# taha-kms/CLASSMATE-RAG

Measured on AMD Instinct MI355X. Metric: hybrid queries/sec + recall@10 vs reference, 10M×768 chunks, 1/2/4/8 GPU, higher is better.
Workload: dtype fp32-accurate E5 (K10 f16x3 MFMA) + int8/f16/f64 dense + f64 BM25

## Files before the change

classmate-rag_amd/classmate_hip/_lib.py:

```python
from __future__ import annotations

import ctypes as C
import os
from pathlib import Path

try:
    import torch
except Exception:
    torch = None

LIB_NAME = "libclassmate_hip.so"
LIB_PATH = Path(os.environ.get("CLASSMATE_HIP_LIB", Path(__file__).with_name(LIB_NAME)))

CM_OK, CM_EINVAL, CM_ENOMEM, CM_EDEVICE, CM_EZERODIV, CM_EUNSUPPORTED = 0, -1, -2, -3, -4, -5
CM_FOP_EQ, CM_FOP_NE, CM_FOP_BITS, CM_FOP_TRUE, CM_FOP_FALSE, CM_FOP_AND, CM_FOP_OR, CM_FOP_NOT = range(1, 9)
CM_FILTER_MAX_OPS, CM_FILTER_MAX_SOURCES = 64, 16
CM_DTYPE_F32, CM_DTYPE_BF16, CM_DTYPE_F16, CM_DTYPE_I32, CM_DTYPE_I64 = 0, 1, 2, 3, 4

if not LIB_PATH.exists():
    raise ImportError(
        f"{LIB_PATH} not found: build the HIP extension first "
        f"(python -c 'import __graft_entry__ as g; g.build()' or make -C classmate-rag_amd)")

lib = C.CDLL(str(LIB_PATH), mode=C.RTLD_GLOBAL)
# ... 66 lines not shown
    "cm_bm25_append": (c_int, c_vp, c_vp, c_vp, c_i64, c_i32),
    "cm_bm25_append_dev": (c_int, c_vp, c_vp, c_vp, c_i64, c_i64, c_i32, c_vp),
    "cm_bm25_remove": (c_int, c_vp, c_vp, c_i64),
    "cm_bm25_remove_dev": (c_int, c_vp, c_vp, c_vp),
    "cm_bm25_replace": (c_int, c_vp, c_vp, c_i64, c_vp, c_vp, c_i32),
    "cm_bm25_replace_dev": (c_int, c_vp, c_vp, c_i64, c_vp, c_vp, c_i64, c_i32, c_vp),
    "cm_bm25_num_docs": (c_i64, c_vp),
    "cm_bm25_num_postings": (c_i64, c_vp),
    "cm_bm25_stats": (c_int, c_vp, P(c_i64), P(c_i64), P(c_f64), P(c_f64)),
    "cm_bm25_export": (c_int, c_vp, c_vp, c_vp, c_vp, c_vp, c_vp),
    "cm_bm25_set_head_policy": (c_int, c_vp, c_f64, c_i64),
    "cm_bm25_num_head_terms": (c_i32, c_vp),
    "cm_bm25_set_path": (c_int, c_vp, c_i32),
    "cm_bm25_workspace_rescored": (c_i32, c_vp, c_i32, c_i32, c_i32, c_vp),
    "cm_bm25_last_rescored": (c_i32, c_vp),
    "cm_bm25_term_stats": (c_int, c_vp, c_vp, c_vp),
    "cm_bm25_set_stats": (c_int, c_vp, c_vp, c_i32, c_i64, c_i64, c_f64),
    "cm_bm25_search": (c_int, c_vp, c_vp, c_vp, c_i32, c_i32, c_vp, c_vp, c_vp, c_vp),
    "cm_bm25_search_lists": (c_int, c_vp, c_vp, c_vp, c_i32, c_i32, c_vp, c_i32, c_vp, c_vp, c_vp, c_vp),
    "cm_bm25_search_lists_dev": (c_int, c_vp, c_vp, c_vp, c_i32, c_i32, c_vp, c_i32, c_vp, c_vp, c_vp, c_vp, c_vp,
                                 c_vp),
    "cm_bm25_last_eps_filters": (c_i32, c_vp),
    "cm_bm25_workspace_items": (c_i64, c_vp, c_i32, c_i32, c_i32, c_vp, c_vp, c_i64),
    "cm_bm25_workspace_subblocks": (c_i64, c_vp, c_i32, c_i32, c_i32, c_vp, c_vp, c_i64),
    "cm_bm25_timing_drain_block": (c_i32, c_vp, c_vp, c_i32),
    "cm_bm25_search_idf": (c_int, c_vp, c_vp, c_vp, c_i32, c_i32, c_vp, c_vp, c_f64, c_i64, c_vp, c_vp, c_vp),
    "cm_bm25_search_workspace": (c_i64, c_vp, c_i32, c_i32, c_i32),
    "cm_bm25_search_dev": (c_int, c_vp, c_vp, c_vp, c_i32, c_i32, c_i32, c_vp, c_vp, c_vp, c_i64, c_vp),
    "cm_bm25_search_dev_gated": (c_int, c_vp, c_vp, c_vp, c_i32, c_i32, c_i32, c_vp, c_vp, c_vp, c_i64, c_vp, c_vp),
    "cm_bm25_prepare_filtered": (c_int, c_vp, c_i64),
    "cm_bm25_filter_stats_dev": (c_int, c_vp, c_vp, c_vp, c_i32, c_vp, c_vp, c_vp),
    "cm_bm25_filter_term_stats_dev": (c_int, c_vp, c_vp, c_vp, c_vp, c_vp),
    "cm_bm25_filter_eps": (c_int, c_vp, c_vp, P(c_f64)),
    "cm_bm25_filter_eps_multi": (c_int, c_vp, c_vp, c_i32, c_vp),
    "cm_bm25_last_eps_passes": (c_i32, c_vp),
    "cm_bm25_search_stats_dev": (c_int, c_vp, c_vp, c_vp, c_i32, c_i32, c_i32, c_vp, c_vp, c_vp, c_vp, c_vp, c_vp,
                                 c_vp, c_vp, c_i64, c_vp),
    "cm_bm25_search_filtered_dev": (c_int, c_vp, c_vp, c_vp, c_i32, c_i32, c_i32, c_vp, c_vp, c_vp, c_vp, c_vp,
                                    c_vp, c_i64, c_vp),
    "cm_mmr": (c_int, c_vp, c_vp, c_vp, c_i32, c_i32, c_i32, c_i32, c_f64, c_vp),
    "cm_mmr_dev": (c_int, c_vp, c_vp, c_vp, c_i32, c_i32, c_i32, c_i32, c_f64, c_vp, c_vp),
    "cm_rrf_fuse": (c_int, c_vp, c_vp, c_i32, c_vp, c_i32, c_vp, c_vp, P(c_i32)),
    "cm_rrf_merge": (c_int, c_vp, c_vp, c_vp, c_i32, c_vp, c_vp, c_vp, c_i32, c_i32, c_f64, c_f64, c_i32, c_i32,
                     c_vp, c_vp, c_vp, c_vp, c_vp, c_vp),
    "cm_rrf_pool_prep_dev": (c_int, c_vp, c_vp, c_i32, c_vp, c_i32, c_vp, c_i32, c_i32, c_vp, c_vp, c_vp, c_vp,
                             c_vp),
# ... 58 lines not shown
```

classmate-rag_amd/classmate_hip/engine.py:

```python
from __future__ import annotations

import ctypes as C
import os
from typing import Optional, Sequence

import numpy as np

from . import _lib as L

try:
    import torch
except Exception:
    torch = None


def default_device() -> int:
    env = os.environ.get("CM_DEVICE")
    if env:
        return int(env)
    if torch is not None and torch.cuda.is_available():
        return torch.cuda.current_device()
    return 0


# ... 459 lines not shown
        L.check(L.fn["cm_bm25_timing"](self._h, int(bool(enable))), "cm_bm25_timing")

    def timing_drain(self, cap: int = 4096) -> list:
        buf = np.zeros(cap, np.float32)
        n = int(L.fn["cm_bm25_timing_drain"](self._h, L.ptr(buf), int(cap)))
        if n < 0:
            raise RuntimeError(L.last_error())
        return buf[:min(n, cap)].tolist()

    def timing_drain_block(self, cap: int = 4096) -> list:
        buf = np.zeros(cap, np.float32)
        n = int(L.fn["cm_bm25_timing_drain_block"](self._h, L.ptr(buf), int(cap)))
        if n < 0:
            raise RuntimeError(L.last_error())
        return buf[:min(n, cap)].tolist()

    def workspace_items(self, nq: int, total_terms: int, k: int, workspace, cap: int = 1 << 22) -> np.ndarray:
        buf = np.zeros(cap, np.uint64)
        n = int(L.fn["cm_bm25_workspace_items"](self._h, int(nq), int(total_terms), int(k), L.ptr(workspace),
                                                 L.ptr(buf), int(cap)))
        if n < 0:
            raise RuntimeError(L.last_error() or "no planned items (full path?)")
        return buf[:min(n, cap)]

    def workspace_subblocks(self, nq: int, total_terms: int, k: int, workspace, cap: int = 1 << 22) -> np.ndarray:
        buf = np.zeros(cap, np.uint64)
        n = int(L.fn["cm_bm25_workspace_subblocks"](self._h, int(nq), int(total_terms), int(k), L.ptr(workspace),
                                                     L.ptr(buf), int(cap)))
        if n < 0:
            raise RuntimeError(L.last_error() or "no planned items (full path?)")
        return buf[:min(n, cap)]

    @property
    def num_head_terms(self) -> int:
        return int(L.fn["cm_bm25_num_head_terms"](self._h))

    def term_stats(self):
        df = np.zeros(max(self.vocab, 1), np.int32)
        fk = np.zeros(max(self.vocab, 1), np.uint64)
        L.check(L.fn["cm_bm25_term_stats"](self._h, L.ptr(df), L.ptr(fk)), "cm_bm25_term_stats")
        return df[: self.vocab], fk[: self.vocab]

    def set_stats(self, idf: np.ndarray, n_live: int, sum_len: int, eps: float):
        v = _c(idf, np.float64)
        L.check(L.fn["cm_bm25_set_stats"](self._h, L.ptr(v), int(v.shape[0]), int(n_live), int(sum_len), float(eps)),
                "cm_bm25_set_stats")
# ... 526 lines not shown
```

classmate-rag_amd/csrc/cm_bm25.hip:

```cpp
#include "cm_common.h"
#include "cm_row_lists.h"

#include <hipcub/hipcub.hpp>

#include <algorithm>
#include <cmath>
#include <cstdlib>
#include <numeric>
#include <vector>

namespace cm {

constexpr int kRange = 1024;
constexpr int kBmThreads = 256;
constexpr int kBoundsGroup = 8;
constexpr int kMergeThreads = 1024;
constexpr int kMergePer = 16;
constexpr int kTermLanesQd = 16;

__device__ inline int64_t lhead(int q, int64_t r, int64_t nr) { return (int64_t)q * nr + r; }
__host__ __device__ inline int64_t lheads_total(int nq, int64_t nr) { return (int64_t)nq * nr; }
__device__ inline int64_t lslot(int q, int64_t r, int64_t nr, int64_t nl, int k, int j) {
  return j == 0 ? lhead(q, r, nr) : nl + ((int64_t)q * nr + r) * (k - 1) + (j - 1);
}
// ... 201 lines not shown
  return __longlong_as_double(((uint64_t)hi << 32) | lo);
}
__device__ inline uint64_t readlane_u64(uint64_t v, int j) {
  const uint32_t lo = __builtin_amdgcn_readlane((uint32_t)v, j);
  const uint32_t hi = __builtin_amdgcn_readlane((uint32_t)(v >> 32), j);
  return ((uint64_t)hi << 32) | lo;
}
__device__ inline void wave_lds_sync() {
  __builtin_amdgcn_fence(__ATOMIC_RELEASE, "wavefront");
  __builtin_amdgcn_wave_barrier();
  __builtin_amdgcn_fence(__ATOMIC_ACQUIRE, "wavefront");
}
template <typename P>
__device__ inline int first_ge(const P *__restrict__ a, int lo, int hi, int32_t target) {
  while (lo < hi) {
    const int mid = (lo + hi) >> 1;
    if (a[mid] < target) lo = mid + 1;
    else hi = mid;
  }
  return lo;
}

template <typename TF>
__global__ void __launch_bounds__(kBmThreads) __attribute__((amdgpu_waves_per_eu(K2_WAVES_PER_EU)))
    bm25_range_kernel(const int32_t *__restrict__ q_terms, const int32_t *__restrict__ q_off, int nq,
                      const double *__restrict__ q_idf, const int64_t *__restrict__ bounds, int nr, int rpw,
                      const int32_t *__restrict__ post_doc, const TF *__restrict__ post_tf,
                      const int32_t *__restrict__ head_id, const uint8_t *__restrict__ headtf, int64_t npad,
                      const int32_t *__restrict__ dl, const uint32_t *__restrict__ live,
                      const uint32_t *__restrict__ allow, int64_t ndocs, const double *__restrict__ avgdl_p,
                      const double *__restrict__ lut, int lut_dmin, int k,
                      uint64_t *__restrict__ cand_key, uint32_t *__restrict__ cand_row,
                      unsigned long long *__restrict__ thr_key, const uint8_t *__restrict__ need, int32_t vocab,
                      int dbg) {
  __shared__ double s_lut[kLutW * kLutTF];
#ifndef CM_ABLATION
  dbg = 0;
#endif
  __shared__ int32_t s_pdoc[kBmThreads / 64][kTailCapW];
  __shared__ uint16_t s_ptf[kBmThreads / 64][kTailCapW];
  __shared__ uint64_t s_keys[kBmThreads / 64][16 * 64];
  const double avgdl = *avgdl_p;
  for (int i = threadIdx.x; i < kLutW * kLutTF; i += kBmThreads) s_lut[i] = lut[i];
  __syncthreads();
  const int lane = threadIdx.x & 63;
  const int wave = threadIdx.x >> 6;
  const int nb = gridDim.x;
  const int b = blockIdx.x;
  const int per = nb >> 3, rem = nb & 7, x = b & 7, y = b >> 3;
  const int lb = (x < rem ? x * (per + 1) : rem * (per + 1) + (x - rem) * per) + y;
  const int nqg = (nq + kQPerWave - 1) / kQPerWave;
  const int wid = lb * (kBmThreads / 64) + wave;
  const int qg = wid % nqg;
  const int q0 = qg * kQPerWave;
  const int rg = wid / nqg;
  const int r0 = rg * rpw, r1 = min(r0 + rpw, nr);
  if (r0 >= r1) return;
  const int nqw = min(kQPerWave, nq - q0);
  auto need_at = [&](int r) -> uint32_t {
    return need ? (uint32_t)__builtin_amdgcn_readfirstlane((int)need[(int64_t)qg * nr + r]) : 0xfu;
  };
  if (need) {
    uint32_t any = 0;
    for (int r = r0; r < r1; ++r) any |= need_at(r);
    if (!any) return;
  }
  int32_t *pdoc = s_pdoc[wave];
  uint16_t *ptf = s_ptf[wave];
  uint64_t *keys = s_keys[wave];
  const int64_t bstride = nr + 1;
  const int my_q = lane / kTermLanes, my_j = lane % kTermLanes;
  int my_tb = 0, my_L = 0;
  if (my_q < nqw) {
    my_tb = q_off[q0 + my_q];
    my_L = q_off[q0 + my_q + 1] - my_tb;
  }
  const bool has_term = my_q < nqw && my_j < my_L;
  const int my_i = my_tb + my_j;
  int32_t my_t = -1, my_h = -1;
  double my_idf = 0.0;
  int64_t my_lo = 0, my_hi = 0;
  if (has_term) {
    my_t = q_terms[my_i];
    if (my_t >= vocab) my_t = -1;
    my_idf = q_idf[my_i];
    my_h = (my_t >= 0 && head_id) ? head_id[my_t] : -1;
    if (my_h < 0) {
      my_lo = bounds[(int64_t)my_i * bstride + r0];
      my_hi = bounds[(int64_t)my_i * bstride + r0 + 1];
    }
  }
  const bool walk = has_term && my_h < 0;
// ... 238 lines not shown
          for (int u = 0; u < 16; ++u) {
            const uint64_t key = keys[u * 64 + lane];
            if (key < bk) {
              bk = key;
              bu = u;
            }
          }
          br = bk == kEmptyKey ? 0xffffffffu : (uint32_t)db + (uint32_t)bu;
        }
      }
      if (lane == 0 && i < k) {
        const int64_t o = lslot(qi, r, nr, lheads_total(nq, nr), k, i);
        cand_key[o] = kEmptyKey;
        cand_row[o] = 0xffffffffu;
      }
      if (i == k && lane == 0 && last < T) atomicMin(thr_key + qi, (unsigned long long)last);
    }
    my_lo = nx_lo;
    my_hi = nx_hi;
    wave_lds_sync();
  }
}

#include "cm_bm25_prune.inc"

__global__ void bm25_head_fill_kernel(const int32_t *__restrict__ head_terms, int nhead,
                                      const int64_t *__restrict__ term_off, const int32_t *__restrict__ post_doc,
                                      const uint16_t *__restrict__ post_tf, uint8_t *__restrict__ headtf,
                                      int64_t npad) {
  const int h = blockIdx.y;
  if (h >= nhead) return;
  const int32_t t = head_terms[h];
  const int64_t lo = term_off[t], hi = term_off[t + 1];
  uint8_t *row = headtf + (int64_t)h * npad;
  for (int64_t p = lo + (int64_t)blockIdx.x * blockDim.x + threadIdx.x; p < hi; p += (int64_t)gridDim.x * blockDim.x)
    row[post_doc[p]] = (uint8_t)post_tf[p];
}

__global__ void bm25_dl_hist_kernel(const int32_t *__restrict__ dl, int64_t ndocs, uint32_t *__restrict__ hist) {
  for (int64_t i = (int64_t)blockIdx.x * blockDim.x + threadIdx.x; i < ndocs; i += (int64_t)gridDim.x * blockDim.x) {
    const int32_t d = dl[i];
    if (d >= 0 && d < 65536) atomicAdd(hist + d, 1u);
  }
}

__global__ void bm25_head_sat_kernel(const int32_t *__restrict__ cand, int ncand, const int64_t *__restrict__ term_off,
// ... 564 lines not shown
  return e ? atoi(e) : 0;
}
#else
int bm25_debug_flags() { return 0; }
#endif

struct BmWs {
  unsigned long long *thr;
  double *lut;
  double *q_idf;
  int64_t *bounds;
  uint64_t *cand_key;
  uint32_t *cand_row;
  uint8_t *need;
  uint64_t *items;
  uint64_t *items_sm;
  uint8_t *qcand;
  int32_t *qd_code;
  double *qd_idf;
  int32_t *qd_tb;
  int32_t *qd_len;
  int32_t *qd_term;
  uint32_t *item_count;
  double *avgdl;
  int64_t *stats;
  int64_t *df;
  size_t total;
};

BmWs bm_ws_layout(const cm_bm25 *h, int nq, int total_terms, int k, void *base) {
  BmWs w{};
  char *p = reinterpret_cast<char *>(base);
  const int64_t nr = std::max<int64_t>(1, ceil_div(h->ndocs, kRange));
  size_t off = 0;
  w.thr = reinterpret_cast<unsigned long long *>(p + off);
  off += round_up((int64_t)std::max(nq, 1) * 8, 256);
  w.lut = reinterpret_cast<double *>(p + off);
  off += round_up((int64_t)kLutW * kLutTF * 8, 256);
  w.q_idf = reinterpret_cast<double *>(p + off);
  off += round_up((int64_t)std::max(total_terms, 1) * 8, 256);
  w.bounds = reinterpret_cast<int64_t *>(p + off);
  off += round_up((int64_t)std::max(total_terms, 1) * (nr + 1) * 8, 256);
  const int64_t n_slots = lheads_total(nq, nr) + (int64_t)nq * nr * (k - 1);
  w.cand_key = reinterpret_cast<uint64_t *>(p + off);
  off += round_up(n_slots * 8, 256);
  w.cand_row = reinterpret_cast<uint32_t *>(p + off);
  off += round_up(n_slots * 4, 256);
  w.need = reinterpret_cast<uint8_t *>(p + off);
  off += round_up(ceil_div(std::max(nq, 1), kQPerWave) * nr, 256);
  w.items = reinterpret_cast<uint64_t *>(p + off);
  off += round_up((int64_t)std::max(nq, 1) * nr * 8, 256);
  w.items_sm = reinterpret_cast<uint64_t *>(p + off);
  off += round_up((int64_t)std::max(nq, 1) * nr * 8, 256);
  w.item_count = reinterpret_cast<uint32_t *>(p + off);
  off += 256;
  w.qcand = reinterpret_cast<uint8_t *>(p + off);
  off += round_up(std::max(total_terms, 1), 256);
  w.avgdl = reinterpret_cast<double *>(p + off);
  off += 256;
  w.stats = reinterpret_cast<int64_t *>(p + off);
  off += 256;
  w.df = reinterpret_cast<int64_t *>(p + off);
  off += round_up((int64_t)std::max(total_terms, 1) * 8, 256);
  w.qd_code = reinterpret_cast<int32_t *>(p + off);
  off += round_up((int64_t)std::max(nq, 1) * kTermLanes * 4, 256);
  w.qd_idf = reinterpret_cast<double *>(p + off);
  off += round_up((int64_t)std::max(nq, 1) * kTermLanes * 8, 256);
  w.qd_tb = reinterpret_cast<int32_t *>(p + off);
  off += round_up((int64_t)std::max(nq, 1) * 4, 256);
  w.qd_len = reinterpret_cast<int32_t *>(p + off);
  off += round_up((int64_t)std::max(nq, 1) * 4, 256);
  w.qd_term = reinterpret_cast<int32_t *>(p + off);
  off += round_up((int64_t)std::max(nq, 1) * kTermLanes * 4, 256);
  w.total = off;
  return w;
}

#ifndef K2A_RPW
// ... 10 lines not shown
                     const uint32_t *allow_dev, const BmWs &w, double *score_dev, int64_t *row_dev, hipStream_t st,
                     hipEvent_t gate = nullptr) {
  int rc;
  const double *avgdl = w.avgdl;
  const int nr = (int)std::max<int64_t>(1, ceil_div(h->ndocs, kRange));
  if (nr > kMergePer * kMergeThreads) CM_FAIL(CM_EUNSUPPORTED, "BM25 shard too large (> 16.7M docs)");
  const int ngroups = (nr + 1 + kBoundsGroup - 1) / kBoundsGroup;
  const int64_t nb = (int64_t)total_terms * ngroups;
  const bool prune = h->path != 1 && !(bm25_debug_flags() & 4);
  if (nq > 0) {
    hipLaunchKernelGGL(bm25_qcand_kernel, dim3((unsigned)ceil_div(nq, 256)), dim3(256), 0, st, q_terms_dev, q_off_dev,
                       nq, h->vocab, h->nhead ? h->head_id.as<int32_t>() : (const int32_t *)nullptr,
                       h->term_off.as<int64_t>(), (int)prune, w.qcand, w.q_idf, prune ? w.qd_code : nullptr,
                       w.qd_idf, w.qd_tb, w.qd_len, w.qd_term);
    CM_HIP(hipGetLastError());
  }
  if (nb > 0) {
    hipLaunchKernelGGL(bm25_bounds_kernel, dim3((unsigned)ceil_div(nb, 256)), dim3(256), 0, st, q_terms_dev,
                       total_terms, h->vocab, nr, h->term_off.as<int64_t>(), h->post_doc.as<int32_t>(), w.qcand,
                       w.bounds);
    CM_HIP(hipGetLastError());
  }
  CM_HIP(hipMemsetAsync(w.thr, 0xff, (size_t)nq * 8, st));
  if (prune && nq > 0 && env_knob("CM_BM25_TSEED", true)) {
    hipLaunchKernelGGL(bm25_tseed_kernel, dim3((unsigned)nq), dim3(kSeedThreads), 0, st, nq, k, w.qd_code,
                       w.qd_idf, w.qd_len, w.qd_term, h->term_off.as<int64_t>(), h->post_doc.as<int32_t>(),
                       h->post_tf.as<uint16_t>(), h->headtf.as<uint8_t>(), h->npad, h->dl.as<int32_t>(),
                       h->live.as<uint32_t>(), allow_dev, avgdl, w.thr);
    CM_HIP(hipGetLastError());
  }
  hipLaunchKernelGGL(bm25_lut_kernel, dim3(kLutW * kLutTF / 256), dim3(256), 0, st, (const double *)avgdl, h->lut_dmin,
                     w.lut);
  CM_HIP(hipGetLastError());
  const int64_t nqg = ceil_div(nq, kQPerWave);
  const int rpw = (int)std::min<int64_t>(kMaxRangesPerWave, std::max<int64_t>(1, nqg * nr / (256 * 4 * 24)));
  const int64_t nwaves = nqg * ceil_div(nr, rpw);
  const int64_t nblk = ceil_div(nwaves, kBmThreads / 64);
  const int rpw_a = std::max(1, std::min(rpw, (int)K2A_RPW));
  const int64_t nblk_a = ceil_div(nqg * ceil_div(nr, rpw_a), K2A_W);
  if (nblk > INT32_MAX || nblk_a > INT32_MAX) CM_FAIL(CM_EUNSUPPORTED, "BM25 batch too large");
  const int32_t *head_id = h->nhead ? h->head_id.as<int32_t>() : (const int32_t *)nullptr;
  if (gate) CM_HIP(hipStreamWaitEvent(st, gate, 0));
#if K2A_TRACE
  if (prune) {
    if ((rc = g_k2a_trace_buf.ensure((size_t)nblk_a * K2A_W * 32))) return rc;
    g_k2a_trace_units = nblk_a * K2A_W;
    uint64_t *tp = g_k2a_trace_buf.as<uint64_t>();
    CM_HIP(hipMemsetAsync(tp, 0, (size_t)g_k2a_trace_units * 32, st));
    CM_HIP(hipMemcpyToSymbolAsync(HIP_SYMBOL(g_k2a_trace), &tp, sizeof(tp), 0, hipMemcpyHostToDevice, st));
  }
#endif
  h->timer.begin(st);
  if (prune) {
    hipLaunchKernelGGL(bm25_tail_kernel<uint16_t>, dim3((unsigned)nblk_a), dim3(64 * K2A_W), 0, st, nq, w.bounds, nr,
                       rpw_a, h->post_doc.as<int32_t>(), h->post_tf.as<uint16_t>(), h->headtf.as<uint8_t>(), h->npad,
                       h->dl.as<int32_t>(), h->live.as<uint32_t>(), allow_dev, avgdl, k, w.cand_key, w.cand_row, w.thr,
                       w.need, w.qd_code, w.qd_term, w.qd_idf, w.qd_tb, w.qd_len, bm25_debug_flags());
    h->timer.end(st);
    CM_HIP(hipGetLastError());
    if ((rc = launch_bm25_merge(w.cand_key, w.cand_row, nq, nr, k, score_dev, row_dev, st))) return rc;
    CM_HIP(hipMemsetAsync(w.item_count, 0, 4, st));
    hipLaunchKernelGGL(bm25_plan_kernel, dim3((unsigned)ceil_div(nqg * nr, 256)), dim3(256), 0, st, w.qd_code,
                       w.qd_idf, w.qd_len, nq, (int)(head_id != nullptr), h->head_maxtf.as<uint8_t>(),
                       h->range_mindl.as<int32_t>(), h->blk_maxtf.as<uint8_t>(), h->blk_mindl.as<int32_t>(),
                       (h->nhead && h->maxr_avgdl > 0.0) ? h->blk_maxr.as<uint8_t>() : (const uint8_t *)nullptr,
                       h->maxr_avgdl, nr, (int64_t)nr * (kRange / 64), avgdl, k, score_dev, row_dev, w.need, w.items,
                       w.item_count,
                       (h->nhead && h->maxr_avgdl > 0.0 && !env_knob("CM_BM25_SUB16_OFF", false))
                           ? h->blk16_maxr.as<uint8_t>() : (const uint8_t *)nullptr,
                       w.items_sm);
    CM_HIP(hipGetLastError());
    h->timer_b.begin(st);
    hipLaunchKernelGGL(bm25_block_kernel, dim3(K2B_GRID), dim3(256), 0, st, w.items, w.item_count, w.qd_code,
                       w.qd_idf, w.qd_tb, w.bounds, nr, h->post_doc.as<int32_t>(), h->headtf.as<uint8_t>(), h->npad,
                       h->dl.as<int32_t>(), h->live.as<uint32_t>(), allow_dev, h->ndocs, avgdl, k, score_dev, nq,
                       w.cand_key, w.cand_row, w.items_sm);
    h->timer_b.end(st);
    CM_HIP(hipGetLastError());
  }
  hipLaunchKernelGGL(bm25_range_kernel<uint16_t>, dim3((unsigned)nblk), dim3(kBmThreads), 0, st, q_terms_dev,
                     q_off_dev, nq, w.q_idf, w.bounds, nr, rpw, h->post_doc.as<int32_t>(),
                     h->post_tf.as<uint16_t>(), head_id, h->headtf.as<uint8_t>(), h->npad, h->dl.as<int32_t>(),
                     h->live.as<uint32_t>(), allow_dev, h->ndocs, avgdl, w.lut, h->lut_dmin, k, w.cand_key,
                     w.cand_row, w.thr, prune ? (const uint8_t *)w.need : (const uint8_t *)nullptr, h->vocab,
                     bm25_debug_flags());
  if (!prune) h->timer.end(st);
  CM_HIP(hipGetLastError());
  return launch_bm25_merge(w.cand_key, w.cand_row, nq, nr, k, score_dev, row_dev, st);
}

int32_t count_rescored(cm_bm25 *h, int nq, const BmWs &w, hipStream_t st) {
  const int64_t nr = std::max<int64_t>(1, ceil_div(h->ndocs, kRange));
  const int64_t n = ceil_div(std::max(nq, 1), kQPerWave) * nr;
  std::vector<uint8_t> v((size_t)n);
  uint32_t items = 0;
  if (hipMemcpyAsync(v.data(), w.need, (size_t)n, hipMemcpyDeviceToHost, st) != hipSuccess ||
      hipMemcpyAsync(&items, w.item_count, 4, hipMemcpyDeviceToHost, st) != hipSuccess ||
      hipStreamSynchronize(st) != hipSuccess)
    return -1;
  int64_t c = items;
  for (uint8_t b : v) c += __builtin_popcount(b);
  return (int32_t)std::min<int64_t>(c, INT32_MAX);
}

void bm25_free(cm_bm25 *h) {
  for (DevBuf *b : {&h->term_off, &h->post_doc, &h->post_tf, &h->post_pos, &h->dl, &h->live, &h->idf, &h->ws,
                    &h->qbuf, &h->obuf, &h->allow_buf, &h->tmp, &h->eps_ws, &h->headtf, &h->head_id, &h->head_maxtf,
                    &h->range_mindl, &h->blk_maxtf, &h->blk_mindl, &h->blk_maxr, &h->blk16_maxr})
// ... 440 lines not shown
  return count_rescored(h, nq, w, h->stream);
}

int32_t cm_bm25_last_rescored(cm_bm25 *h) { return h ? h->last_rescored : -1; }

int64_t cm_bm25_workspace_items(cm_bm25 *h, int32_t nq, int32_t total_terms, int32_t k, const void *workspace_dev,
                                uint64_t *items_out, int64_t cap) {
  if (!h || !workspace_dev || nq <= 0 || k <= 0 || cap < 0) return -1;
  if (h->path == 1) return -1;
  DeviceGuard dg(h->dev);
  const BmWs w = bm_ws_layout(h, nq, total_terms, k, const_cast<void *>(workspace_dev));
  uint32_t n = 0;
  if (hipMemcpyAsync(&n, w.item_count, 4, hipMemcpyDeviceToHost, h->stream) != hipSuccess ||
      hipStreamSynchronize(h->stream) != hipSuccess)
    return -1;
  const int64_t m = std::min<int64_t>(n, cap);
  if (m > 0 && items_out &&
      (hipMemcpyAsync(items_out, w.items, (size_t)m * 8, hipMemcpyDeviceToHost, h->stream) != hipSuccess ||
       hipStreamSynchronize(h->stream) != hipSuccess))
    return -1;
  return n;
}

int64_t cm_bm25_workspace_subblocks(cm_bm25 *h, int32_t nq, int32_t total_terms, int32_t k, const void *workspace_dev,
                                    uint64_t *masks_out, int64_t cap) {
  if (!h || !workspace_dev || nq <= 0 || k <= 0 || cap < 0) return -1;
  if (h->path == 1) return -1;
  DeviceGuard dg(h->dev);
  const BmWs w = bm_ws_layout(h, nq, total_terms, k, const_cast<void *>(workspace_dev));
  uint32_t n = 0;
  if (hipMemcpyAsync(&n, w.item_count, 4, hipMemcpyDeviceToHost, h->stream) != hipSuccess ||
      hipStreamSynchronize(h->stream) != hipSuccess)
    return -1;
  const int64_t m = std::min<int64_t>(n, cap);
  if (m > 0 && masks_out &&
      (hipMemcpyAsync(masks_out, w.items_sm, (size_t)m * 8, hipMemcpyDeviceToHost, h->stream) != hipSuccess ||
       hipStreamSynchronize(h->stream) != hipSuccess))
    return -1;
  return n;
}

#if K2A_TRACE
int64_t cm_bm25_k2a_trace(cm_bm25 *h, uint64_t *out, int64_t cap_units) {
  if (!h || !out) return -1;
  DeviceGuard dg(h->dev);
  if (hipDeviceSynchronize() != hipSuccess) return -1;
// ... 357 lines not shown
```

classmate-rag_amd/csrc/cm_bm25_prune.inc:

```

#ifndef K2A_CAP
#define K2A_CAP 320
#endif
#ifndef K2A_SUB
#define K2A_SUB 4
#endif
#ifndef K2B_U
#define K2B_U 2
#endif
#ifndef K2A_WPE
#define K2A_WPE 5
#endif
#ifndef K2A_W
#define K2A_W 1
#endif

#ifndef K2A_TRACE
#define K2A_TRACE 0
#endif
#if K2A_TRACE
__device__ uint64_t *g_k2a_trace;
#endif
typedef uint16_t u16x2_t __attribute__((ext_vector_type(2)));
constexpr int kCandCap = K2A_CAP;
// ... 336 lines not shown
    r += nsub;
  }
#if K2A_TRACE
  if (lane == 0) {
    uint64_t *tr = g_k2a_trace + 4 * (int64_t)wid;
    const uint64_t xcc = __builtin_amdgcn_s_getreg((3 << 11) | 20) & 15u;
    tr[0] = (xcc << 32) | (uint64_t)(wid + 1);
    tr[1] = tr_t0;
    tr[2] = __builtin_amdgcn_s_memrealtime();
    tr[3] = tr_post;
  }
#endif
}

__global__ void __launch_bounds__(256)
    bm25_plan_kernel(const int32_t *__restrict__ qd_code, const double *__restrict__ qd_idf,
                     const int32_t *__restrict__ qd_len, int nq, int has_heads,
                     const uint8_t *__restrict__ head_maxtf, const int32_t *__restrict__ range_mindl,
                     const uint8_t *__restrict__ blk_maxtf, const int32_t *__restrict__ blk_mindl,
                     const uint8_t *__restrict__ blk_maxr, double maxr_avgdl, int nr,
                     int64_t nblk, const double *__restrict__ avgdl_p, int k, const double *__restrict__ top_score,
                     const int64_t *__restrict__ top_row, uint8_t *__restrict__ need, uint64_t *__restrict__ items,
                     uint32_t *__restrict__ item_count, const uint8_t *__restrict__ blk16_maxr,
                     uint64_t *__restrict__ items_sm) {
  const double avgdl = *avgdl_p;
  const bool use_r = blk_maxr != nullptr && avgdl <= maxr_avgdl;
  const float inv_avg = inv_avg_lo(avgdl);
  auto kd_lo = [&](int32_t dlen) __attribute__((always_inline)) { return kd_lo32(dlen, inv_avg); };
  const int nqg = (nq + kQPerWave - 1) / kQPerWave;
  const int64_t gid = (int64_t)blockIdx.x * blockDim.x + threadIdx.x;
  const bool act = gid < (int64_t)nqg * nr;
  const int lane = threadIdx.x & 63;
  uint64_t it[kQPerWave], its[kQPerWave];
  int nit = 0;
  if (act) {
    const int qg = (int)(gid / nr), r = (int)(gid - (int64_t)qg * nr);
    uint32_t m = need[gid];
    const float kd = kd_lo(range_mindl[r]);
    for (int qq = 0; qq < kQPerWave; ++qq) {
      const int q = qg * kQPerWave + qq;
      if (q >= nq) break;
      const uint32_t bit = 1u << qq;
      if (m & bit) continue;
      const double T = top_score[(int64_t)q * k + k - 1];
      if (qd_len[q] > kTermLanes || top_row[(int64_t)q * k + k - 1] < 0 || !(T > 0.0)) {
        m |= bit;
        continue;
      }
      if (!has_heads) continue;
      int32_t hs[kTermLanes];
      float fi[kTermLanes];
      uint32_t mt[kTermLanes];
      {
        const int4 *cp = reinterpret_cast<const int4 *>(qd_code + (int64_t)q * kTermLanes);
        const double2 *ip = reinterpret_cast<const double2 *>(qd_idf + (int64_t)q * kTermLanes);
#pragma unroll
        for (int v = 0; v < kTermLanes / 4; ++v) {
// ... 89 lines not shown
        if ((double)(ubb[b] * kPlanSlack) >= T) bm |= 1u << b;
      uint64_t sm = 0;
#pragma unroll
      for (int b = 0; b < 16; ++b) {
        if (!((bm >> b) & 1u)) continue;
        if (!use_s) {
          sm |= 0xfull << (4 * b);
          continue;
        }
#pragma unroll
        for (int x = 0; x < 4; ++x)
          if ((double)(ubs[4 * b + x] * kPlanSlack) >= T) sm |= 1ull << (4 * b + x);
      }
      uint32_t bms = 0;
#pragma unroll
      for (int b = 0; b < 16; ++b)
        if ((sm >> (4 * b)) & 0xfull) bms |= 1u << b;
      if (bms) {
        its[nit] = sm;
        it[nit++] = ((uint64_t)q << 40) | ((uint64_t)r << 16) | bms;
      }
    }
    need[gid] = (uint8_t)m;
  }
  int incl = nit;
#pragma unroll
  for (int o = 1; o < 64; o <<= 1) {
    const int v = __shfl_up(incl, o);
    if (lane >= o) incl += v;
  }
  const int total = __shfl(incl, 63);
  if (total == 0) return;
  uint32_t base = 0;
  if (lane == 63) base = atomicAdd(item_count, (uint32_t)total);
  base = (uint32_t)__shfl((int)base, 63);
  for (int i = 0; i < nit; ++i) {
    items[base + (uint32_t)(incl - nit + i)] = it[i];
    items_sm[base + (uint32_t)(incl - nit + i)] = its[i];
  }
}

__device__ inline bool k2b_below(const uint32_t (&tfv)[kTermLanes], float fi, float kd, double T, uint64_t headm) {
  float ub = 0.0f;
#pragma unroll
  for (int j = 0; j < kTermLanes; ++j)
    if ((headm >> j) & 1u) ub += __int_as_float(__builtin_amdgcn_readlane(__float_as_int(fi), j)) * ratio_up32(tfv[j], kd);
// ... 456 lines not shown
```

include/classmate_hip.h:

```cpp
#ifndef CLASSMATE_HIP_H
#define CLASSMATE_HIP_H

#include <stddef.h>
#include <stdint.h>

#ifdef __cplusplus
extern "C" {
#endif

#define CM_OK 0
#define CM_EINVAL (-1)
#define CM_ENOMEM (-2)
#define CM_EDEVICE (-3)
#define CM_EZERODIV (-4)
#define CM_EUNSUPPORTED (-5)

#define CM_DTYPE_F32 0
#define CM_DTYPE_BF16 1
#define CM_DTYPE_F16 2
#define CM_DTYPE_I32 3
#define CM_DTYPE_I64 4

const char *cm_last_error(void);
int cm_version(void);
// ... 72 lines not shown
int cm_bm25_append(cm_bm25 *h, const int32_t *term_ids, const int64_t *doc_off, int64_t n_new, int32_t vocab);
int cm_bm25_append_dev(cm_bm25 *h, const int32_t *term_ids_dev, const int64_t *doc_off_dev, int64_t n_new,
                       int64_t ntokens, int32_t vocab, void *stream);
int cm_bm25_remove(cm_bm25 *h, const int64_t *rows, int64_t n_rows);
int cm_bm25_remove_dev(cm_bm25 *h, const uint32_t *remove_bits_dev, void *stream);
int cm_bm25_replace(cm_bm25 *h, const int64_t *rows, int64_t n_rows, const int32_t *term_ids, const int64_t *doc_off,
                    int32_t vocab);
int cm_bm25_replace_dev(cm_bm25 *h, const int64_t *rows_dev, int64_t n_rows, const int32_t *term_ids_dev,
                        const int64_t *doc_off_dev, int64_t ntokens, int32_t vocab, void *stream);
int64_t cm_bm25_num_docs(cm_bm25 *h);
int64_t cm_bm25_num_postings(cm_bm25 *h);
int cm_bm25_stats(cm_bm25 *h, int64_t *n_live, int64_t *sum_len, double *avgdl, double *eps);
int cm_bm25_set_head_policy(cm_bm25 *h, double min_df_frac, int64_t max_bytes);
int32_t cm_bm25_num_head_terms(cm_bm25 *h);
#define CM_BM25_FULL 1
#define CM_BM25_PRUNED 2
int cm_bm25_set_path(cm_bm25 *h, int32_t kind);
int32_t cm_bm25_workspace_rescored(cm_bm25 *h, int32_t nq, int32_t total_terms, int32_t k, const void *workspace_dev);
int32_t cm_bm25_last_rescored(cm_bm25 *h);
int64_t cm_bm25_workspace_items(cm_bm25 *h, int32_t nq, int32_t total_terms, int32_t k, const void *workspace_dev,
                                uint64_t *items_out, int64_t cap);
int64_t cm_bm25_workspace_subblocks(cm_bm25 *h, int32_t nq, int32_t total_terms, int32_t k, const void *workspace_dev,
                                    uint64_t *masks_out, int64_t cap);
int cm_bm25_timing(cm_bm25 *h, int32_t enable);
int32_t cm_bm25_timing_drain(cm_bm25 *h, float *ms_out, int32_t cap);
int32_t cm_bm25_timing_drain_block(cm_bm25 *h, float *ms_out, int32_t cap);
int cm_bm25_export(cm_bm25 *h, int64_t *term_off, int32_t *post_doc, uint16_t *post_tf, uint32_t *post_pos,
                   int32_t *dl);
int cm_bm25_term_stats(cm_bm25 *h, int32_t *df_out, uint64_t *first_out);
int cm_bm25_set_stats(cm_bm25 *h, const double *idf, int32_t vocab, int64_t n_live, int64_t sum_len, double eps);
int cm_bm25_search(cm_bm25 *h, const int32_t *q_terms, const int32_t *q_off, int32_t nq, int32_t k,
                   const uint32_t *allow_bits, double *out_score, int64_t *out_row, int32_t *out_n);
int cm_bm25_search_lists(cm_bm25 *h, const int32_t *q_terms, const int32_t *q_off, int32_t nq, int32_t k,
                         const uint32_t *allow_bits, int32_t n_filters, const int32_t *filter_of,
                         double *out_score, int64_t *out_row, int32_t *out_n);
int cm_bm25_search_lists_dev(cm_bm25 *h, const int32_t *q_terms, const int32_t *q_off, int32_t nq, int32_t k,
                             const uint32_t *allow_bits, int32_t n_filters, const int32_t *filter_of, double *eps_io,
                             double *score_dev, int64_t *row_dev, int32_t *out_n, void *stream);
int32_t cm_bm25_last_eps_filters(cm_bm25 *h);
int cm_bm25_search_idf(cm_bm25 *h, const int32_t *q_terms, const int32_t *q_off, int32_t nq, int32_t k,
                       const uint32_t *allow_bits, const double *q_idf, double avgdl, int64_t n_cand,
                       double *out_score, int64_t *out_row, int32_t *out_n);
int64_t cm_bm25_search_workspace(cm_bm25 *h, int32_t nq, int32_t total_terms, int32_t k);
int cm_bm25_search_dev(cm_bm25 *h, const int32_t *q_terms_dev, const int32_t *q_off_dev, int32_t nq,
                       int32_t total_terms, int32_t k, double *score_dev, int64_t *row_dev,
                       void *workspace_dev, int64_t workspace_bytes, void *stream);
// ... 95 lines not shown
```

Before: 35220.

## Compact needed BM25 ranges into a work list for the range kernel

The plan kernel now appends every (query-group, range) pair whose need mask is nonzero to a compact device list via wave-ballot atomics. The range kernel gains a LIST variant that launches a fixed grid and has waves grid-stride over only the listed pairs, instead of launching one wave per pair and early-exiting on empty ones. This is meant to remove launch and scheduling cost for the many pruned-away ranges and to balance work better. In exchange it adds an atomic counter, extra workspace, and one range per list entry, which loses the multi-range-per-wave batching.

After: 35390 (median of 6 runs). About the same (+0.5%).

```diff
diff --git a/classmate-rag_amd/classmate_hip/_lib.py b/classmate-rag_amd/classmate_hip/_lib.py
--- a/classmate-rag_amd/classmate_hip/_lib.py
+++ b/classmate-rag_amd/classmate_hip/_lib.py
@@ -112,6 +112,7 @@
                                  c_vp),
     "cm_bm25_last_eps_filters": (c_i32, c_vp),
     "cm_bm25_workspace_items": (c_i64, c_vp, c_i32, c_i32, c_i32, c_vp, c_vp, c_i64),
+    "cm_bm25_workspace_need_ranges": (c_i64, c_vp, c_i32, c_i32, c_i32, c_vp, c_vp, c_vp, c_i64),
     "cm_bm25_workspace_subblocks": (c_i64, c_vp, c_i32, c_i32, c_i32, c_vp, c_vp, c_i64),
     "cm_bm25_timing_drain_block": (c_i32, c_vp, c_vp, c_i32),
     "cm_bm25_search_idf": (c_int, c_vp, c_vp, c_vp, c_i32, c_i32, c_vp, c_vp, c_f64, c_i64, c_vp, c_vp, c_vp),
diff --git a/classmate-rag_amd/classmate_hip/engine.py b/classmate-rag_amd/classmate_hip/engine.py
--- a/classmate-rag_amd/classmate_hip/engine.py
+++ b/classmate-rag_amd/classmate_hip/engine.py
@@ -505,6 +505,17 @@
         if n < 0:
             raise RuntimeError(L.last_error() or "no planned items (full path?)")
         return buf[:min(n, cap)]
+
+    def workspace_need_ranges(self, nq: int, total_terms: int, k: int, workspace, detail: bool = False):
+        nqg, nr = (int(nq) + 3) // 4, max(1, (self.num_docs + 1023) // 1024)
+        lst = np.zeros(nqg * nr, np.uint32)
+        need = np.zeros(nqg * nr, np.uint8)
+        n = int(L.fn["cm_bm25_workspace_need_ranges"](self._h, int(nq), int(total_terms), int(k), L.ptr(workspace),
+                                                      L.ptr(lst) if detail else None,
+                                                      L.ptr(need) if detail else None, nqg * nr))
+        if n < 0:
+            raise RuntimeError(L.last_error() or "no need list (full path?)")
+        return (n, lst[:min(n, nqg * nr)], need.reshape(nqg, nr)) if detail else n
 
     def workspace_subblocks(self, nq: int, total_terms: int, k: int, workspace, cap: int = 1 << 22) -> np.ndarray:
         buf = np.zeros(cap, np.uint64)
diff --git a/classmate-rag_amd/csrc/cm_bm25.hip b/classmate-rag_amd/csrc/cm_bm25.hip
--- a/classmate-rag_amd/csrc/cm_bm25.hip
+++ b/classmate-rag_amd/csrc/cm_bm25.hip
@@ -247,52 +247,23 @@
 }
 
 template <typename TF>
-__global__ void __launch_bounds__(kBmThreads) __attribute__((amdgpu_waves_per_eu(K2_WAVES_PER_EU)))
-    bm25_range_kernel(const int32_t *__restrict__ q_terms, const int32_t *__restrict__ q_off, int nq,
-                      const double *__restrict__ q_idf, const int64_t *__restrict__ bounds, int nr, int rpw,
-                      const int32_t *__restrict__ post_doc, const TF *__restrict__ post_tf,
-                      const int32_t *__restrict__ head_id, const uint8_t *__restrict__ headtf, int64_t npad,
-                      const int32_t *__restrict__ dl, const uint32_t *__restrict__ live,
-                      const uint32_t *__restrict__ allow, int64_t ndocs, const double *__restrict__ avgdl_p,
-                      const double *__restrict__ lut, int lut_dmin, int k,
-                      uint64_t *__restrict__ cand_key, uint32_t *__restrict__ cand_row,
-                      unsigned long long *__restrict__ thr_key, const uint8_t *__restrict__ need, int32_t vocab,
-                      int dbg) {
-  __shared__ double s_lut[kLutW * kLutTF];
-#ifndef CM_ABLATION
-  dbg = 0;
-#endif
-  __shared__ int32_t s_pdoc[kBmThreads / 64][kTailCapW];
-  __shared__ uint16_t s_ptf[kBmThreads / 64][kTailCapW];
-  __shared__ uint64_t s_keys[kBmThreads / 64][16 * 64];
-  const double avgdl = *avgdl_p;
-  for (int i = threadIdx.x; i < kLutW * kLutTF; i += kBmThreads) s_lut[i] = lut[i];
-  __syncthreads();
+__device__ __forceinline__ void
+    bm25_range_body(const int qg, const int r0, const int r1, const double *s_lut, int32_t *pdoc, uint16_t *ptf,
+                    uint64_t *keys, const double avgdl, const int32_t *__restrict__ q_terms,
+                    const int32_t *__restrict__ q_off, int nq, const double *__restrict__ q_idf,
+                    const int64_t *__restrict__ bounds, int nr, const int32_t *__restrict__ post_doc,
+                    const TF *__restrict__ post_tf, const int32_t *__restrict__ head_id,
+                    const uint8_t *__restrict__ headtf, int64_t npad, const int32_t *__restrict__ dl,
+                    const uint32_t *__restrict__ live, const uint32_t *__restrict__ allow, int64_t ndocs,
+                    int lut_dmin, int k, uint64_t *__restrict__ cand_key, uint32_t *__restrict__ cand_row,
+                    unsigned long long *__restrict__ thr_key, const uint8_t *__restrict__ need, int32_t vocab,
+                    int dbg) {
   const int lane = threadIdx.x & 63;
-  const int wave = threadIdx.x >> 6;
-  const int nb = gridDim.x;
-  const int b = blockIdx.x;
-  const int per = nb >> 3, rem = nb & 7, x = b & 7, y = b >> 3;
-  const int lb = (x < rem ? x * (per + 1) : rem * (per + 1) + (x - rem) * per) + y;
-  const int nqg = (nq + kQPerWave - 1) / kQPerWave;
-  const int wid = lb * (kBmThreads / 64) + wave;
-  const int qg = wid % nqg;
   const int q0 = qg * kQPerWave;
-  const int rg = wid / nqg;
-  const int r0 = rg * rpw, r1 = min(r0 + rpw, nr);
-  if (r0 >= r1) return;
   const int nqw = min(kQPerWave, nq - q0);
   auto need_at = [&](int r) -> uint32_t {
     return need ? (uint32_t)__builtin_amdgcn_readfirstlane((int)need[(int64_t)qg * nr + r]) : 0xfu;
   };
-  if (need) {
-    uint32_t any = 0;
-    for (int r = r0; r < r1; ++r) any |= need_at(r);
-    if (!any) return;
-  }
-  int32_t *pdoc = s_pdoc[wave];
-  uint16_t *ptf = s_ptf[wave];
-  uint64_t *keys = s_keys[wave];
   const int64_t bstride = nr + 1;
   const int my_q = lane / kTermLanes, my_j = lane % kTermLanes;
   int my_tb = 0, my_L = 0;
@@ -577,6 +548,68 @@
   }
 }
 
+#ifndef K2_LIST_GRID
+#define K2_LIST_GRID 512
+#endif
+template <typename TF, bool LIST>
+__global__ void __launch_bounds__(kBmThreads) __attribute__((amdgpu_waves_per_eu(K2_WAVES_PER_EU)))
+    bm25_range_kernel(const int32_t *__restrict__ q_terms, const int32_t *__restrict__ q_off, int nq,
+                      const double *__restrict__ q_idf, const int64_t *__restrict__ bounds, int nr, int rpw,
+                      const int32_t *__restrict__ post_doc, const TF *__restrict__ post_tf,
+                      const int32_t *__restrict__ head_id, const uint8_t *__restrict__ headtf, int64_t npad,
+                      const int32_t *__restrict__ dl, const uint32_t *__restrict__ live,
+                      const uint32_t *__restrict__ allow, int64_t ndocs, const double *__restrict__ avgdl_p,
+                      const double *__restrict__ lut, int lut_dmin, int k,
+                      uint64_t *__restrict__ cand_key, uint32_t *__restrict__ cand_row,
+                      unsigned long long *__restrict__ thr_key, const uint8_t *__restrict__ need, int32_t vocab,
+                      int dbg, const uint32_t *__restrict__ need_list, const uint32_t *__restrict__ need_count) {
+  __shared__ double s_lut[kLutW * kLutTF];
+#ifndef CM_ABLATION
+  dbg = 0;
+#endif
+  __shared__ int32_t s_pdoc[kBmThreads / 64][kTailCapW];
+  __shared__ uint16_t s_ptf[kBmThreads / 64][kTailCapW];
+  __shared__ uint64_t s_keys[kBmThreads / 64][16 * 64];
+  uint32_t n_list = 0;
+  if (LIST) {
+    n_list = *need_count;
+    if (blockIdx.x * (uint32_t)(kBmThreads / 64) >= n_list) return;
+  }
+  const double avgdl = *avgdl_p;
+  for (int i = threadIdx.x; i < kLutW * kLutTF; i += kBmThreads) s_lut[i] = lut[i];
+  __syncthreads();
+  const int wave = threadIdx.x >> 6;
+  if (LIST) {
+    const uint32_t stride = gridDim.x * (uint32_t)(kBmThreads / 64);
+    for (uint32_t e = blockIdx.x * (uint32_t)(kBmThreads / 64) + (uint32_t)wave; e < n_list; e += stride) {
+      const uint32_t g = (uint32_t)__builtin_amdgcn_readfirstlane((int)need_list[e]);
+      const int qg = (int)(g / (uint32_t)nr), r0 = (int)(g % (uint32_t)nr);
+      bm25_range_body<TF>(qg, r0, r0 + 1, s_lut, s_pdoc[wave], s_ptf[wave], s_keys[wave], avgdl, q_terms, q_off, nq,
+                          q_idf, bounds, nr, post_doc, post_tf, head_id, headtf, npad, dl, live, allow, ndocs,
+                          lut_dmin, k, cand_key, cand_row, thr_key, need, vocab, dbg);
+    }
+    return;
+  }
+  const int nb = gridDim.x;
+  const int b = blockIdx.x;
+  const int per = nb >> 3, rem = nb & 7, x = b & 7, y = b >> 3;
+  const int lb = (x < rem ? x * (per + 1) : rem * (per + 1) + (x - rem) * per) + y;
+  const int nqg = (nq + kQPerWave - 1) / kQPerWave;
+  const int wid = lb * (kBmThreads / 64) + wave;
+  const int qg = wid % nqg;
+  const int rg = wid / nqg;
+  const int r0 = rg * rpw, r1 = min(r0 + rpw, nr);
+  if (r0 >= r1) return;
+  if (need) {
+    uint32_t any = 0;
+    for (int r = r0; r < r1; ++r) any |= (uint32_t)__builtin_amdgcn_readfirstlane((int)need[(int64_t)qg * nr + r]);
+    if (!any) return;
+  }
+  bm25_range_body<TF>(qg, r0, r1, s_lut, s_pdoc[wave], s_ptf[wave], s_keys[wave], avgdl, q_terms, q_off, nq, q_idf,
+                      bounds, nr, post_doc, post_tf, head_id, headtf, npad, dl, live, allow, ndocs, lut_dmin, k,
+                      cand_key, cand_row, thr_key, need, vocab, dbg);
+}
+
 #include "cm_bm25_prune.inc"
 
 __global__ void bm25_head_fill_kernel(const int32_t *__restrict__ head_terms, int nhead,
@@ -1187,6 +1220,8 @@
   int32_t *qd_len;
   int32_t *qd_term;
   uint32_t *item_count;
+  uint32_t *need_count;
+  uint32_t *need_list;
   double *avgdl;
   int64_t *stats;
   int64_t *df;
@@ -1218,7 +1253,10 @@
   w.items_sm = reinterpret_cast<uint64_t *>(p + off);
   off += round_up((int64_t)std::max(nq, 1) * nr * 8, 256);
   w.item_count = reinterpret_cast<uint32_t *>(p + off);
+  w.need_count = w.item_count + 1;
   off += 256;
+  w.need_list = reinterpret_cast<uint32_t *>(p + off);
+  off += round_up(ceil_div(std::max(nq, 1), kQPerWave) * nr * 4, 256);
   w.qcand = reinterpret_cast<uint8_t *>(p + off);
   off += round_up(std::max(total_terms, 1), 256);
   w.avgdl = reinterpret_cast<double *>(p + off);
@@ -1275,6 +1313,7 @@
     CM_HIP(hipGetLastError());
   }
   CM_HIP(hipMemsetAsync(w.thr, 0xff, (size_t)nq * 8, st));
+  if (prune) CM_HIP(hipMemsetAsync(w.item_count, 0, 8, st));
   if (prune && nq > 0 && env_knob("CM_BM25_TSEED", true)) {
     hipLaunchKernelGGL(bm25_tseed_kernel, dim3((unsigned)nq), dim3(kSeedThreads), 0, st, nq, k, w.qd_code,
                        w.qd_idf, w.qd_len, w.qd_term, h->term_off.as<int64_t>(), h->post_doc.as<int32_t>(),
@@ -1291,7 +1330,8 @@
   const int64_t nblk = ceil_div(nwaves, kBmThreads / 64);
   const int rpw_a = std::max(1, std::min(rpw, (int)K2A_RPW));
   const int64_t nblk_a = ceil_div(nqg * ceil_div(nr, rpw_a), K2A_W);
-  if (nblk > INT32_MAX || nblk_a > INT32_MAX) CM_FAIL(CM_EUNSUPPORTED, "BM25 batch too large");
+  if (nblk > INT32_MAX || nblk_a > INT32_MAX || nqg * nr > (int64_t)UINT32_MAX)
+    CM_FAIL(CM_EUNSUPPORTED, "BM25 batch too large");
   const int32_t *head_id = h->nhead ? h->head_id.as<int32_t>() : (const int32_t *)nullptr;
   if (gate) CM_HIP(hipStreamWaitEvent(st, gate, 0));
 #if K2A_TRACE
@@ -1312,7 +1352,6 @@
     h->timer.end(st);
     CM_HIP(hipGetLastError());
     if ((rc = launch_bm25_merge(w.cand_key, w.cand_row, nq, nr, k, score_dev, row_dev, st))) return rc;
-    CM_HIP(hipMemsetAsync(w.item_count, 0, 4, st));
     hipLaunchKernelGGL(bm25_plan_kernel, dim3((unsigned)ceil_div(nqg * nr, 256)), dim3(256), 0, st, w.qd_code,
                        w.qd_idf, w.qd_len, nq, (int)(head_id != nullptr), h->head_maxtf.as<uint8_t>(),
                        h->range_mindl.as<int32_t>(), h->blk_maxtf.as<uint8_t>(), h->blk_mindl.as<int32_t>(),
@@ -1321,7 +1360,7 @@
                        w.item_count,
                        (h->nhead && h->maxr_avgdl > 0.0 && !env_knob("CM_BM25_SUB16_OFF", false))
                            ? h->blk16_maxr.as<uint8_t>() : (const uint8_t *)nullptr,
-                       w.items_sm);
+                       w.items_sm, w.need_list, w.need_count);
     CM_HIP(hipGetLastError());
     h->timer_b.begin(st);
     hipLaunchKernelGGL(bm25_block_kernel, dim3(K2B_GRID), dim3(256), 0, st, w.items, w.item_count, w.qd_code,
@@ -1331,12 +1370,20 @@
     h->timer_b.end(st);
     CM_HIP(hipGetLastError());
   }
-  hipLaunchKernelGGL(bm25_range_kernel<uint16_t>, dim3((unsigned)nblk), dim3(kBmThreads), 0, st, q_terms_dev,
-                     q_off_dev, nq, w.q_idf, w.bounds, nr, rpw, h->post_doc.as<int32_t>(),
-                     h->post_tf.as<uint16_t>(), head_id, h->headtf.as<uint8_t>(), h->npad, h->dl.as<int32_t>(),
-                     h->live.as<uint32_t>(), allow_dev, h->ndocs, avgdl, w.lut, h->lut_dmin, k, w.cand_key,
-                     w.cand_row, w.thr, prune ? (const uint8_t *)w.need : (const uint8_t *)nullptr, h->vocab,
-                     bm25_debug_flags());
+  if (prune && env_knob("CM_BM25_NEED_LIST", true))
+    hipLaunchKernelGGL((bm25_range_kernel<uint16_t, true>), dim3(K2_LIST_GRID), dim3(kBmThreads), 0, st, q_terms_dev,
+                       q_off_dev, nq, w.q_idf, w.bounds, nr, 1, h->post_doc.as<int32_t>(),
+                       h->post_tf.as<uint16_t>(), head_id, h->headtf.as<uint8_t>(), h->npad, h->dl.as<int32_t>(),
+                       h->live.as<uint32_t>(), allow_dev, h->ndocs, avgdl, w.lut, h->lut_dmin, k, w.cand_key,
+                       w.cand_row, w.thr, (const uint8_t *)w.need, h->vocab, bm25_debug_flags(),
+                       (const uint32_t *)w.need_list, (const uint32_t *)w.need_count);
+  else
+    hipLaunchKernelGGL((bm25_range_kernel<uint16_t, false>), dim3((unsigned)nblk), dim3(kBmThreads), 0, st,
+                       q_terms_dev, q_off_dev, nq, w.q_idf, w.bounds, nr, rpw, h->post_doc.as<int32_t>(),
+                       h->post_tf.as<uint16_t>(), head_id, h->headtf.as<uint8_t>(), h->npad, h->dl.as<int32_t>(),
+                       h->live.as<uint32_t>(), allow_dev, h->ndocs, avgdl, w.lut, h->lut_dmin, k, w.cand_key,
+                       w.cand_row, w.thr, prune ? (const uint8_t *)w.need : (const uint8_t *)nullptr, h->vocab,
+                       bm25_debug_flags(), (const uint32_t *)nullptr, (const uint32_t *)nullptr);
   if (!prune) h->timer.end(st);
   CM_HIP(hipGetLastError());
   return launch_bm25_merge(w.cand_key, w.cand_row, nq, nr, k, score_dev, row_dev, st);
@@ -1823,6 +1870,27 @@
   return n;
 }
 
+int64_t cm_bm25_workspace_need_ranges(cm_bm25 *h, int32_t nq, int32_t total_terms, int32_t k,
+                                      const void *workspace_dev, uint32_t *list_out, uint8_t *need_out, int64_t cap) {
+  if (!h || !workspace_dev || nq <= 0 || k <= 0 || cap < 0) return -1;
+  if (h->path == 1) return -1;
+  DeviceGuard dg(h->dev);
+  const BmWs w = bm_ws_layout(h, nq, total_terms, k, const_cast<void *>(workspace_dev));
+  const int64_t pairs = ceil_div(nq, kQPerWave) * std::max<int64_t>(1, ceil_div(h->ndocs, kRange));
+  uint32_t n = 0;
+  if (hipMemcpyAsync(&n, w.need_count, 4, hipMemcpyDeviceToHost, h->stream) != hipSuccess ||
+      hipStreamSynchronize(h->stream) != hipSuccess)
+    return -1;
+  const int64_t m = std::min<int64_t>(std::min<int64_t>(n, pairs), cap), mb = std::min(pairs, cap);
+  if ((m > 0 && list_out &&
+       hipMemcpyAsync(list_out, w.need_list, (size_t)m * 4, hipMemcpyDeviceToHost, h->stream) != hipSuccess) ||
+      (mb > 0 && need_out &&
+       hipMemcpyAsync(need_out, w.need, (size_t)mb, hipMemcpyDeviceToHost, h->stream) != hipSuccess) ||
+      hipStreamSynchronize(h->stream) != hipSuccess)
+    return -1;
+  return n;
+}
+
 int64_t cm_bm25_workspace_subblocks(cm_bm25 *h, int32_t nq, int32_t total_terms, int32_t k, const void *workspace_dev,
                                     uint64_t *masks_out, int64_t cap) {
   if (!h || !workspace_dev || nq <= 0 || k <= 0 || cap < 0) return -1;
diff --git a/classmate-rag_amd/csrc/cm_bm25_prune.inc b/classmate-rag_amd/csrc/cm_bm25_prune.inc
--- a/classmate-rag_amd/csrc/cm_bm25_prune.inc
+++ b/classmate-rag_amd/csrc/cm_bm25_prune.inc
@@ -382,7 +382,8 @@
                      int64_t nblk, const double *__restrict__ avgdl_p, int k, const double *__restrict__ top_score,
                      const int64_t *__restrict__ top_row, uint8_t *__restrict__ need, uint64_t *__restrict__ items,
                      uint32_t *__restrict__ item_count, const uint8_t *__restrict__ blk16_maxr,
-                     uint64_t *__restrict__ items_sm) {
+                     uint64_t *__restrict__ items_sm, uint32_t *__restrict__ need_list,
+                     uint32_t *__restrict__ need_count) {
   const double avgdl = *avgdl_p;
   const bool use_r = blk_maxr != nullptr && avgdl <= maxr_avgdl;
   const float inv_avg = inv_avg_lo(avgdl);
@@ -393,6 +394,7 @@
   const int lane = threadIdx.x & 63;
   uint64_t it[kQPerWave], its[kQPerWave];
   int nit = 0;
+  bool listed = false;
   if (act) {
     const int qg = (int)(gid / nr), r = (int)(gid - (int64_t)qg * nr);
     uint32_t m = need[gid];
@@ -528,6 +530,14 @@
       }
     }
     need[gid] = (uint8_t)m;
+    listed = m != 0;
+  }
+  const uint64_t lm = __ballot(listed);
+  if (lm) {
+    uint32_t lbase = 0;
+    if (lane == 0) lbase = atomicAdd(need_count, (uint32_t)__popcll(lm));
+    lbase = (uint32_t)__builtin_amdgcn_readfirstlane((int)lbase);
+    if (listed) need_list[lbase + (uint32_t)__popcll(lm & ((1ull << lane) - 1))] = (uint32_t)gid;
   }
   int incl = nit;
 #pragma unroll
diff --git a/include/classmate_hip.h b/include/classmate_hip.h
--- a/include/classmate_hip.h
+++ b/include/classmate_hip.h
@@ -118,6 +118,8 @@
                                 uint64_t *items_out, int64_t cap);
 int64_t cm_bm25_workspace_subblocks(cm_bm25 *h, int32_t nq, int32_t total_terms, int32_t k, const void *workspace_dev,
                                     uint64_t *masks_out, int64_t cap);
+int64_t cm_bm25_workspace_need_ranges(cm_bm25 *h, int32_t nq, int32_t total_terms, int32_t k,
+                                      const void *workspace_dev, uint32_t *list_out, uint8_t *need_out, int64_t cap);
 int cm_bm25_timing(cm_bm25 *h, int32_t enable);
 int32_t cm_bm25_timing_drain(cm_bm25 *h, float *ms_out, int32_t cap);
 int32_t cm_bm25_timing_drain_block(cm_bm25 *h, float *ms_out, int32_t cap);
```
